# yinan-codes/Rossby-wave-ray-tracing

Measured on AMD Instinct MI355X. Metric: ray-steps/sec (whole node), 10^6 rays RKF45; max |Δpos| vs CPU ref, higher is better.
Workload: dtype f64

## Files before the change

### include/rwrt.h

```cpp
#ifndef RWRT_H
#define RWRT_H

#include <stdint.h>

#ifdef __cplusplus
extern "C" {
#endif

#define RWRT_ABI_VERSION 5
#define RWRT_NFIELD_REF 18
#define RWRT_NFIELD_PACK 12
#define RWRT_NVAR 5
#define RWRT_NMERC 12
#define RWRT_NOUT 8
#define RWRT_NSTATE 12

typedef enum {
  RWRT_OK = 0,
  RWRT_ERR_ARG = 1,
  RWRT_ERR_HIP = 2,
  RWRT_SOLVER_FAILED = 3
} rwrt_status;

typedef struct {
// ... 87 lines not shown
                                int64_t nray, const rwrt_params* p,
                                const double* d_tbound, int32_t it_begin,
                                int32_t it_end, const int64_t* d_order,
                                int64_t n_heavy, double* d_state, int64_t* d_count,
                                int32_t* d_nanrow, double* d_out, int32_t* d_tail_from,
                                double* d_tail_row, int32_t* d_work, void* stream);
rwrt_status rwrt_expand_tails(int64_t nray, int32_t it_begin, int32_t it_end,
                              const int32_t* d_tail_from, const double* d_tail_row,
                              double* d_out, void* stream);

rwrt_status rwrt_row_slots(int64_t nray, const double* d_state, int32_t* d_row_slot, int64_t* d_nslot,
                           void* stream);
rwrt_status rwrt_rk45_run_slots(rwrt_ctx* ctx, const rwrt_grid* g, const double* d_packed,
                                int64_t nray, const rwrt_params* p,
                                const double* d_tbound, int32_t it_begin,
                                int32_t it_end, const int64_t* d_order,
                                int64_t n_heavy, double* d_state, int64_t* d_count,
                                int32_t* d_nanrow, double* d_out, const int32_t* d_row_slot,
                                int32_t* d_tail_from, double* d_tail_row, int32_t* d_work,
                                void* stream);
rwrt_status rwrt_expand_slots(int64_t nray, int32_t it_begin, int32_t it_end, const int32_t* d_row_slot,
                              const int32_t* d_tail_from, const double* d_tail_row, const double* d_rows,
                              double* d_out, void* stream);

typedef struct {
  int32_t nx, ny, nchan, wcol;
  double inv_dlon;
  double lat0, inv_dlat;
} rwrt_density_map;

rwrt_status rwrt_ray_density(const rwrt_density_map* m, int64_t nray,
                             int32_t it_begin, int32_t it_end,
                             const double* d_rows, const int32_t* d_row_slot,
                             const int32_t* d_tail_from, const double* d_tail_row,
                             const int32_t* d_chan, int64_t* d_count, double* d_wsum,
                             void* stream);

#define RWRT_SUMMARY_MAXREG 8
#define RWRT_SUMMARY_NF64 9
#define RWRT_SUMMARY_NI32 4
typedef struct {
  int32_t nreg, reserved;
  double box[RWRT_SUMMARY_MAXREG][4];
} rwrt_summary_regions;

rwrt_status rwrt_ray_summary(int64_t nray, int32_t it_begin, int32_t it_end,
// ... 143 lines not shown
```

### rossby-wave-ray-tracing_amd/_hip.py

```python
import ctypes
import os

import torch

_HERE = os.path.dirname(os.path.abspath(__file__))
LIB_PATH = os.environ.get("RWRT_LIB", os.path.join(_HERE, "librwrt.so"))

NFIELD_REF, NFIELD_PACK, NVAR, NMERC, NOUT, NSTATE = 18, 12, 5, 12, 8, 12
ABI_SYMBOLS = ("rwrt_version", "rwrt_last_error", "rwrt_ctx_create", "rwrt_ctx_destroy",
               "rwrt_ctx_set_latency_density", "rwrt_ctx_set_tv_lanes", "rwrt_ctx_set_handoff",
               "rwrt_ctx_set_trace",
               "rwrt_pack_fields",
               "rwrt_mercator_point", "rwrt_rhs", "rwrt_dp54_attempt",
               "rwrt_ray_initial", "rwrt_rk45_init", "rwrt_rk45_run", "rwrt_rk45_run_tails",
               "rwrt_expand_tails", "rwrt_row_slots", "rwrt_rk45_run_slots", "rwrt_expand_slots",
               "rwrt_rk4_run", "rwrt_ray_density", "rwrt_ray_summary", "rwrt_ray_arrival", "rwrt_ray_flux",
               "rwrt_ray_track", "rwrt_ray_cross",
               "rwrt_wn_map", "rwrt_wn_fill",
               "rwrt_sh_filter",
               "rwrt_bs_ready", "rwrt_bs_diag", "rwrt_rk45_init_tv", "rwrt_rk45_run_tv", "rwrt_rk45_run_tv_tails",
               "rwrt_rk45_run_tv_slots", "rwrt_rhs_tv",
               "rwrt_kat_rk45", "rwrt_selftest_math", "rwrt_host_fill_rows")

RWRT_OK, RWRT_ERR_ARG, RWRT_ERR_HIP, RWRT_SOLVER_FAILED = 0, 1, 2, 3


class RwrtError(RuntimeError):
    pass


class SolverFailed(RwrtError):
    """rkf45.py:423-425: every retrying column has a NaN step (status -1)."""


class Grid(ctypes.Structure):
    _fields_ = [("ncol", ctypes.c_int32), ("nrow", ctypes.c_int32),
                ("lon0", ctypes.c_double), ("dlon", ctypes.c_double),
                ("lat0", ctypes.c_double), ("dlat", ctypes.c_double)]


class Params(ctypes.Structure):
    _fields_ = [("rtol", ctypes.c_double), ("atol", ctypes.c_double),
                ("min_step", ctypes.c_double), ("cut_off", ctypes.c_double),
                ("nt", ctypes.c_int32), ("reserved", ctypes.c_int32),
                ("tstep", ctypes.c_double)]


# ... 76 lines not shown
    lib.rwrt_last_error.restype = ctypes.c_char_p
    G, Pr, B = ctypes.POINTER(Grid), ctypes.POINTER(Params), ctypes.POINTER(Background)
    M = ctypes.POINTER(DensityMap)
    R = ctypes.POINTER(SummaryRegions)
    A = ctypes.POINTER(ArrivalMap)
    F = ctypes.POINTER(FluxMapC)
    T = ctypes.POINTER(TrackMapC)
    X = ctypes.POINTER(CrossMapC)
    sig = {
        "rwrt_pack_fields": [G, _P, _P, _P],
        "rwrt_mercator_point": [G, _P, _I64, _P, _P, _P, _P],
        "rwrt_rhs": [G, _P, _I64, _P, _P, _P],
        "rwrt_dp54_attempt": [G, _P, _I64, _P, _P, _P, _D, _D, _P, _P, _P, _P],
        "rwrt_ray_initial": [G, _P, _I64, _P, _P, _P, _I32, _P, _P, _P, _P],
        "rwrt_rk45_init": [G, _P, _I64, _P, Pr, _P, _P, _P, _P, _P, _P],
        "rwrt_rk45_run": [_P, G, _P, _I64, Pr, _P, _I32, _I32, _P, _I64, _P, _P, _P, _P, _P, _P],
        "rwrt_rk45_run_tails": [_P, G, _P, _I64, Pr, _P, _I32, _I32, _P, _I64, _P, _P, _P, _P, _P, _P, _P,
                                _P],
        "rwrt_expand_tails": [_I64, _I32, _I32, _P, _P, _P, _P],
        "rwrt_row_slots": [_I64, _P, _P, _P, _P],
        "rwrt_rk45_run_slots": [_P, G, _P, _I64, Pr, _P, _I32, _I32, _P, _I64, _P, _P, _P, _P, _P, _P, _P,
                                _P, _P],
        "rwrt_expand_slots": [_I64, _I32, _I32, _P, _P, _P, _P, _P, _P],
        "rwrt_rk4_run": [_P, G, _P, _I64, Pr, _I32, _I32, _P, _P, _P, _P, _P, _P, _P],
        "rwrt_ray_density": [M, _I64, _I32, _I32, _P, _P, _P, _P, _P, _P, _P, _P],
        "rwrt_ray_arrival": [A, _I64, _I32, _I32, _P, _P, _P, _P, _P, _P, _P, _P, _P],
        "rwrt_ray_flux": [F, _I64, _I32, _I32, _P, _P, _P, _P, _P, _P, _P, _P],
        "rwrt_ray_track": [T, _I64, _I32, _I32, _P, _P, _P, _P, _P, _I64, _P, _P, _P, _P, _P, _P, _P],
        "rwrt_ray_cross": [X, _I64, _I32, _I32, _P, _P, _P, _P, _P, _I64, _P, _P, _P, _P, _P, _P, _P, _P, _P],
        "rwrt_ray_summary": [_I64, _I32, _I32, _P, _P, _P, _P, _P, _I64, R, _P, _P, _P],
        "rwrt_wn_map": [G, _P, _I32, _I64, _I32, _P, _P, _P, _I32, _P, _P, _P, _P, _P, _P, _P],
        "rwrt_wn_fill": [_I32, _I32, _I32, _I32, _P, _P, _P],
        "rwrt_sh_filter": [_I32, _I32, _I32, _I32, _P, _P, _P, _P, _P, _P, _P, _P],
        "rwrt_bs_ready": [_I32, _I32, _P, _P, _P, _D, _D, _P, _P, _I32, _P],
        "rwrt_bs_diag": [_I32, _I32, _I32, _P, _P, _P, _D, _D, ctypes.c_uint32, _P, _P, _I32, _P],
        "rwrt_rk45_init_tv": [G, B, _I64, _P, Pr, _P, _P, _P, _P, _P, _P],
        "rwrt_rk45_run_tv": [_P, G, B, _I64, Pr, _P, _I32, _I32, _P, _I64, _P, _P, _P, _P, _P, _P],
        "rwrt_rk45_run_tv_tails": [_P, G, B, _I64, Pr, _P, _I32, _I32, _P, _I64, _P, _P, _P, _P, _P, _P, _P,
                                   _P],
        "rwrt_rk45_run_tv_slots": [_P, G, B, _I64, Pr, _P, _I32, _I32, _P, _I64, _P, _P, _P, _P, _P, _P, _P,
                                   _P, _P],
        "rwrt_ctx_create": [_I32, ctypes.POINTER(_P)],
        "rwrt_ctx_destroy": [_P],
        "rwrt_ctx_set_latency_density": [_P, _I32],
        "rwrt_ctx_set_tv_lanes": [_P, _I32],
        "rwrt_ctx_set_handoff": [_P, _I32],
# ... 61 lines not shown

    def set_latency_density(self, rays_per_wave):
        if getattr(self, "_qpw", 16) != int(rays_per_wave):
            check(load().rwrt_ctx_set_latency_density(self._h, int(rays_per_wave)))
            self._qpw = int(rays_per_wave)

    def set_tv_lanes(self, lanes):
        if getattr(self, "_tvl", 64) != int(lanes):
            check(load().rwrt_ctx_set_tv_lanes(self._h, int(lanes)))
            self._tvl = int(lanes)

    def set_handoff(self, max_rays):
        if getattr(self, "_hof", 16) != int(max_rays):
            check(load().rwrt_ctx_set_handoff(self._h, int(max_rays)))
            self._hof = int(max_rays)

    def set_trace(self, trace=None):
        if trace is None:
            check(load().rwrt_ctx_set_trace(self._h, None, 0))
        else:
            check(load().rwrt_ctx_set_trace(self._h, ctypes.c_void_p(trace.data_ptr()), int(trace.shape[0])))
        self._trace = trace

    def close(self):
        h, self._h = getattr(self, "_h", None), None
        if h is not None and h.value and _lib is not None:
            _lib.rwrt_ctx_destroy(h)

    def __del__(self):
        try:
            self.close()
        except Exception:
            pass
```

### rossby-wave-ray-tracing_amd/csrc/rwrt.hip

```cpp

#include <hip/hip_runtime.h>

#include <cmath>
#include <cstdint>
#include <cstdlib>
#include <cstdio>
#include <cstring>
#include <mutex>
#include <string>
#include <type_traits>

#include "rwrt.h"
#include "nproots.h"

#ifdef RWRT_ANALYZE_HOT
__device__ __forceinline__ bool rwrt_rare_sink(bool c) {
  asm volatile("; rare %0" ::"s"(__builtin_amdgcn_ballot_w64(c)));
  return false;
}
#define RARE(c) rwrt_rare_sink(c)
#else
#define RARE(c) (c)
#endif
#ifdef RWRT_ANALYZE_MARK
// ... 2036 lines not shown
  double cut_a;
  const uint8_t* frozen;
  int32_t quad_per_wave = 16;
  int64_t* trace = nullptr;
  int64_t trace_cap = 0;
  const int32_t* row_slot = nullptr;
  int32_t handoff = 16;
};

template <class BG>
__device__ __forceinline__ double* row_block(const RunArgs<BG>& a, int64_t ray) {
  const int64_t slot = a.row_slot ? (int64_t)a.row_slot[ray] : ray;
  return slot < 0 ? nullptr : a.out + (size_t)slot * (size_t)(a.it_end - a.it_begin) * RWRT_NOUT;
}


__device__ __forceinline__ void store_tail(double* tail_row, int64_t ray, double2 r0, double2 r1, double2 r2,
                                           double2 r3) {
  double2* o = reinterpret_cast<double2*>(tail_row + (size_t)ray * RWRT_NOUT);
  o[0] = r0;
  o[1] = r1;
  o[2] = r2;
  o[3] = r3;
}

constexpr int kTraceWords = 10;
__device__ __forceinline__ void trace_start(int64_t* tr, int64_t w) {
  tr[w * kTraceWords + 3] = (int64_t)__builtin_amdgcn_s_memrealtime();
  tr[w * kTraceWords + 8] = (int64_t)__builtin_amdgcn_s_memtime();
}
__device__ __forceinline__ void trace_ray(int64_t* tr, int64_t w, int64_t ray, int64_t attempts, bool latency) {
  const unsigned hw = __builtin_amdgcn_s_getreg(4 | (31 << 11));
  const unsigned xcc = __builtin_amdgcn_s_getreg(20 | (15 << 11));
  int64_t* r = tr + w * kTraceWords;
  r[0] = ray;
  r[1] = hw;
  r[2] = xcc;
  r[4] = (int64_t)__builtin_amdgcn_s_memrealtime();
  r[5] = attempts;
  r[6] = latency ? 1 : 0;
  r[7] = blockIdx.x;
  r[9] = (int64_t)__builtin_amdgcn_s_memtime();
}

inline double haversine_cut(double cut_off) {
  if (!(cut_off > 0.0 && cut_off <= 3.0)) return -1.0;
// ... 327 lines not shown
      ug = aux[0];
      vg = aux[1];
    } else {
      ugvg_at(a.B, tb, y[0], y[1], y[2], y[3], ug, vg);
    }
    const int last = (st == 2) ? a.it_end : it + 1;
    if (writer && rows) {
      const double2 r0 = make_double2(y[0], y[1]), r1 = make_double2(y[2], y[3]);
      const double2 r2 = make_double2(y[4], ug), r3 = make_double2(vg, (double)nacc);
      for (int kr = it; kr < last; ++kr) {
        double2* o = reinterpret_cast<double2*>(rows + (size_t)(kr - a.it_begin) * RWRT_NOUT);
        store_row16<RWRT_ROW_NT>(o + 0, r0);
        store_row16<RWRT_ROW_NT>(o + 1, r1);
        store_row16<RWRT_ROW_NT>(o + 2, r2);
        store_row16<RWRT_ROW_NT>(o + 3, r3);
      }
    }
    if (nanrow == a.nt && isnan(y[0])) nanrow = it;
    prev_lon = y[0];
    prev_lat = y[1];
    cos_prev = cos_c;
    it = last;
    if (st == 2) t = a.tbound[a.it_end - 1];
    if (it == a.it_end) break;
  }
  if (writer) {
#pragma unroll
    for (int v = 0; v < 5; ++v) {
      a.state[v * a.nray + ray] = y[v];
      a.state[(5 + v) * a.nray + ray] = f[v];
    }
    a.state[10 * a.nray + ray] = t;
    a.state[11 * a.nray + ray] = habs;
    a.count[2 * ray] = nacc;
    a.count[2 * ray + 1] = nrej;
    a.nanrow[ray] = nanrow;
    if (kTrace && w < a.trace_cap) trace_ray(a.trace, w, ray, nacc + nrej - att0, true);
  }
}

template <bool kTrace>
__device__ __forceinline__ void quad_rays(const RunArgs<StaticBG>& a, char* cache, double* Kq, int lb) {
  const CachedStaticBG B = LaneBG<StaticBG>::make(a.B, cache);
  QuadRole R;
  R.role = threadIdx.x & 3;
  R.odd = (R.role & 1) != 0;
  R.high = (R.role & 2) != 0;
// ... 140 lines not shown
      double2* o = reinterpret_cast<double2*>(rows + (size_t)(it - a.it_begin) * RWRT_NOUT);
      store_row16<RWRT_ROW_NT>(o + 0, r0);
      store_row16<RWRT_ROW_NT>(o + 1, r1);
      store_row16<RWRT_ROW_NT>(o + 2, r2);
      store_row16<RWRT_ROW_NT>(o + 3, r3);
    }
    if (RARE(last > it + 1) && writer && rows) {
      asm volatile("");
      for (int k = it + 1; k < last; ++k) {
        double2* o = reinterpret_cast<double2*>(rows + (size_t)(k - a.it_begin) * RWRT_NOUT);
        o[0] = r0;
        o[1] = r1;
        o[2] = r2;
        o[3] = r3;
      }
    }
    if (nanrow == a.nt && isnan(y[0])) nanrow = it;
    prev_lon = y[0];
    prev_lat = y[1];
    cos_prev = cos_c;
    it = last;
    if (st == Lane<RayProblem, KStore>::kFrozen) L.t = a.tbound[a.it_end - 1];
    if (it == a.it_end && writer) {
#pragma unroll
      for (int v = 0; v < 5; ++v) {
        a.state[v * a.nray + ray] = y[v];
        a.state[(5 + v) * a.nray + ray] = L.f[v];
      }
      a.state[10 * a.nray + ray] = L.t;
      a.state[11 * a.nray + ray] = L.habs;
      if (kTrace && wpos < a.trace_cap)
        trace_ray(a.trace, wpos, ray, nacc + nrej - a.count[2 * ray] - a.count[2 * ray + 1], false);
      a.count[2 * ray] = nacc;
      a.count[2 * ray + 1] = nrej;
      a.nanrow[ray] = nanrow;
      ray = -1;
    }
    if ((kReplica || kPair) && it == a.it_end) ray = -1;
    MARK("x_row_end_done");
  }
  if constexpr (kHandoff) {
    const uint64_t hm = __builtin_amdgcn_ballot_w64(handoff);
    if (RARE(hm != 0)) {
      const int q = (int)((threadIdx.x & 63u) >> 2);
      const int nq = __builtin_popcountll(hm);
      uint64_t m = hm;
// ... 64 lines not shown
      run_rays<BG, BBG, false, true>(a, BBG::make(a.B, smem + kKBytes), smem, w);
      return;
    }
  }
  if constexpr (std::is_same<BG, VaryingBG<double>>::value) {
#ifdef RWRT_ANALYZE_PAIR
    if (true) {
#else
    if (a.B.half) {
#endif
      run_rays<BG, PairVaryingBG64, false, false, true>(a, PairVaryingBG64::make(a.B, smem + kKBytes), smem, -1);
      return;
    }
  }
  if constexpr (kLean)
    run_rays<BG, LeanCachedStaticBG, kTrace, false>(a, LeanCachedStaticBG{LaneBG<BG>::make(a.B, smem + kKBytes)}, smem,
                                                    -1);
  else
    run_rays<BG, typename LaneBG<BG>::type, kTrace, false>(a, LaneBG<BG>::make(a.B, smem + kKBytes), smem, -1);
}

__global__ void frozen_flag_kernel(const double* __restrict__ state, int64_t nray,
                                   uint8_t* __restrict__ frozen, int32_t* __restrict__ tail_from = nullptr,
                                   int32_t it_begin = 0, int32_t it_end = 0) {
  for (int64_t i = blockIdx.x * (int64_t)blockDim.x + threadIdx.x; i < nray;
       i += (int64_t)gridDim.x * blockDim.x) {
    double sum = state[i];
#pragma unroll
    for (int v = 1; v < 5; ++v) sum = sum + state[v * nray + i];
    const bool frz = isnan(sum / 5.0);
    frozen[i] = frz ? 1 : 0;
    if (tail_from) tail_from[i] = frz ? it_begin : it_end;
  }
}

constexpr int kFillThreads = 64;
__device__ __forceinline__ void write_frozen_tile(double* out, int64_t base, int64_t nrows, bool mine,
                                                  double2 r0, double2 r1, double2 r2, double2 r3) {
  unsigned long long lanes = __ballot(mine);
  const int64_t nq = nrows * 4;
  const int qt = threadIdx.x & 3;
  while (lanes) {
    const int j = __builtin_ctzll(lanes);
    lanes &= lanes - 1;
    double2* o = reinterpret_cast<double2*>(out + (size_t)(base + j) * nrows * RWRT_NOUT);
    const double2 q0 = make_double2(__shfl(r0.x, j), __shfl(r0.y, j));
    const double2 q1 = make_double2(__shfl(r1.x, j), __shfl(r1.y, j));
// ... 472 lines not shown

struct DeviceGuard {
  int prev = -1;
  bool ok = true;
  explicit DeviceGuard(int dev) {
    if (hipGetDevice(&prev) != hipSuccess) prev = -1;
    if (prev != dev) ok = hipSetDevice(dev) == hipSuccess;
  }
  ~DeviceGuard() {
    int cur = -1;
    if (prev >= 0 && hipGetDevice(&cur) == hipSuccess && cur != prev) (void)hipSetDevice(prev);
  }
};

rwrt_status ctx_flags(rwrt_ctx* c, int64_t nray) {
  if ((size_t)nray <= c->cap) return RWRT_OK;
  if (c->flags) {
    if ((c->used && hipEventSynchronize(c->done) != hipSuccess) || hipFree(c->flags) != hipSuccess)
      return check_launch("releasing the context's frozen-ray flags");
    c->flags = nullptr;
    c->cap = 0;
  }
  const size_t cap = ((size_t)nray + 4095) & ~(size_t)4095;
  if (hipMalloc(reinterpret_cast<void**>(&c->flags), cap) != hipSuccess)
    return fail(RWRT_ERR_HIP, "frozen-ray flag allocation failed%s");
  c->cap = cap;
  return RWRT_OK;
}

rwrt_status ctx_image(rwrt_ctx* c, const Field& F, hipStream_t stream, const char** out,
                      const int** range = nullptr) {
  const size_t image = cache_image_bytes((int64_t)F.W * F.H), need = image + kRangeInts * sizeof(int);
  if (need > c->img_cap) {
    if (c->img) {
      if ((c->used && hipEventSynchronize(c->done) != hipSuccess) || hipFree(c->img) != hipSuccess)
        return check_launch("releasing the context's cache image");
      c->img = nullptr;
      c->img_cap = 0;
    }
    if (hipMalloc(reinterpret_cast<void**>(&c->img), need) != hipSuccess)
      return fail(RWRT_ERR_HIP, "cache image allocation failed%s");
    c->img_cap = need;
  }
  int* r = reinterpret_cast<int*>(c->img + image);
  if (hipMemsetAsync(r, 0, kRangeInts * sizeof(int), stream) != hipSuccess)
    return check_launch("hipMemsetAsync(exponent range)");
  hipLaunchKernelGGL(cache_image_kernel, dim3(grid_for((int64_t)F.W * F.H * 6, 256)), dim3(256), 0, stream,
// ... 68 lines not shown
  const int32_t quad_per_wave = ctx->quad_per_wave;
  const int32_t handoff = ctx->handoff;
  const int64_t per_block = BG::kTimeVarying ? 4 : 4 * (int64_t)quad_per_wave;
  const int64_t team_blocks = (n_heavy + per_block - 1) / per_block;
  if (team_blocks > ctx->ncu / 2)
    return fail(RWRT_ERR_ARG, "n_heavy exceeds the latency mode's capacity (per CU 4 x rays-per-wave, time-varying 4; half the CUs)%s");
  DeviceGuard dg(ctx->device);
  if (!dg.ok) return check_launch("hipSetDevice(context device)");
  hipStream_t st = (hipStream_t)stream;
  if (hipMemsetAsync(d_work, 0, 2 * sizeof(int32_t), st) != hipSuccess)
    return check_launch("hipMemsetAsync(queue)");
  int64_t blocks = ctx_persistent_blocks<BG>(ctx);
  if (team_blocks) blocks = std::max<int64_t>(1, blocks - team_blocks * (blocks / ctx->ncu));
  int64_t block_rays = 256;
  if constexpr (BG::kTimeVarying) block_rays = B.half ? 128 : 256;
  const int64_t need = (nray - n_heavy + block_rays - 1) / block_rays;
  if (blocks > need) blocks = need;
  RunArgs<BG> a{B, nray, p->rtol, p->atol, p->min_step, p->cut_off, p->nt, it_begin, it_end,
                d_tbound, d_order, d_state, d_count, d_nanrow, d_out, d_work,
                n_heavy, 0, haversine_cut(p->cut_off), nullptr};
  a.row_slot = d_row_slot;
  a.handoff = handoff;
  if (rwrt_status s = ctx_flags(ctx, nray)) return s;
  a.frozen = ctx->flags;
  if (rwrt_status s = ctx_begin(ctx, st, [&] {
        hipLaunchKernelGGL(frozen_flag_kernel, dim3(grid_for(nray, 256)), dim3(256), 0, st, d_state, nray,
                           ctx->flags, d_tail_from, it_begin, it_end);
      }))
    return s;
  if constexpr (std::is_same<BG, StaticBG>::value) {
    if (rwrt_status s = ctx_image(ctx, B.F, st, &a.B.img, &a.B.range)) return s;
  }
  a.heavy_blocks = (int32_t)team_blocks;
  a.quad_per_wave = quad_per_wave;
  if constexpr (std::is_same<BG, StaticBG>::value) {
    a.trace = ctx->trace;
    a.trace_cap = ctx->trace ? ctx->trace_cap : 0;
  }
  if (nray > n_heavy || team_blocks) {
    const int64_t grid = team_blocks + (nray > n_heavy ? blocks : 0);
    if (a.trace && std::is_same<BG, StaticBG>::value) {
      if constexpr (std::is_same<BG, StaticBG>::value) {
        hipLaunchKernelGGL((rk45_run_kernel<BG, true>), dim3((unsigned)grid), dim3(256), 0, st, a);
        hipLaunchKernelGGL((rk45_run_kernel<BG, true, true>), dim3((unsigned)grid), dim3(256), 0, st, a);
      }
    } else {
      hipLaunchKernelGGL(rk45_run_kernel<BG>, dim3((unsigned)grid), dim3(256), 0, st, a);
      if constexpr (std::is_same<BG, StaticBG>::value)
        hipLaunchKernelGGL((rk45_run_kernel<BG, false, true>), dim3((unsigned)grid), dim3(256), 0, st, a);
    }
// ... 748 lines not shown
```

### rossby-wave-ray-tracing_amd/engine.py

```python
import os

import numpy as np
import torch

import _hip as H
from constants import rearth as R_EARTH
from launch_rows import deliver

F64 = torch.float64


def grid_of(lon, lat, ncol):
    lon = np.asarray(lon, np.float64)
    lat = np.asarray(lat, np.float64)
    return H.Grid(int(ncol), len(lat), float(lon[0]), float(lon[1] - lon[0]),
                  float(lat[0]), float(lat[1] - lat[0]))


def t_eval_of(nt, tstep, ttotal=None):
    t = np.arange(nt) * np.float64(tstep)
    if ttotal is not None and t[-1] > ttotal:
        t[-1] = ttotal
    return t


class RunResult:

    def __init__(self, nacc, nrej, nanrow, failed, break_row, n_live):
        self.nacc = nacc
        self.nrej = nrej
        self.nanrow = nanrow
        self.failed = failed
        self.break_row = break_row
        self.n_live = n_live
        self.bounds = []

    @property
    def ray_steps(self):
        return int(self.nacc.sum().item())


class Tails:

    def __init__(self, nray, device):
        self.frm = torch.empty(nray, dtype=torch.int32, device=device)
        self.row = torch.empty((nray, H.NOUT), dtype=F64, device=device)

    def take(self, idx):
        t = Tails.__new__(Tails)
        t.frm, t.row = self.frm[idx].contiguous(), self.row[idx].contiguous()
        return t

    def last_row(self, view, i1):
        return torch.where((self.frm < i1)[:, None], self.row, view[:, -1])


class Slots:

    def __init__(self, nray, device):
        self.slot = torch.empty(nray, dtype=torch.int32, device=device)
        self.n_dev = torch.zeros(1, dtype=torch.int64, device=device)
        self.n = None

    def compute(self, st, stream):
        H.check(H.load().rwrt_row_slots(st["nray"], H.dptr(st["state"]), H.dptr(self.slot, torch.int32),
                                        H.dptr(self.n_dev, torch.int64), stream))
        return self

    def count(self):
        self.n = int(self.n_dev.item())
        return self.n

    def last_row(self, view, tails, i1):
        blk = view[self.slot.clamp(min=0).to(torch.int64), -1] if view.shape[0] else tails.row
        return torch.where((tails.frm < i1)[:, None], tails.row, blk)

    def dense(self, view, tails, i0, i1, out=None):
        nray = self.slot.numel()
        if out is None or out.numel() < nray * (i1 - i0) * H.NOUT:
            out = torch.empty((nray, i1 - i0, H.NOUT), dtype=F64, device=self.slot.device)
        d = out.reshape(-1)[: nray * (i1 - i0) * H.NOUT].view(nray, i1 - i0, H.NOUT)
        H.check(H.load().rwrt_expand_slots(nray, int(i0), int(i1), H.dptr(self.slot, torch.int32),
                                           H.dptr(tails.frm, torch.int32), H.dptr(tails.row, F64),
                                           H.dptr(view, F64), H.dptr(d, F64), H.stream(self.slot.device)))
        return d


class RayEngine:

    use_tails = os.environ.get("RWRT_TAILS", "1") != "0"
    tv_lanes = int(os.environ.get("RWRT_TV_LANES", "32"))
    use_slots = os.environ.get("RWRT_SLOTS", "1") != "0"
    handoff = int(os.environ.get("RWRT_HANDOFF", "16"))

    def __init__(self, fields, lon, lat, device=None):
        H.require_gpu()
        H.load()
        self.device = torch.device(device or "cuda")
        f = torch.as_tensor(np.ascontiguousarray(fields, dtype=np.float64)) \
            if not torch.is_tensor(fields) else fields.to(F64)
        if f.ndim != 3 or f.shape[-1] != H.NFIELD_REF:
            raise ValueError(f"fields must be [ncol, nrow, {H.NFIELD_REF}], got {tuple(f.shape)}")
        f = f.to(self.device).contiguous()
        self.grid = grid_of(lon, lat, f.shape[0])
        self.lon, self.lat = np.array(lon, np.float64), np.array(lat, np.float64)
        self.packed = torch.empty((f.shape[0], f.shape[1], H.NFIELD_PACK), dtype=F64,
                                  device=self.device)
        H.check(H.load().rwrt_pack_fields(self.grid, H.dptr(f), H.dptr(self.packed), self._stream()))
        self.work = torch.zeros(4, dtype=torch.int32, device=self.device)

    bg = None
    split_rho = None
    launch_log = ()
    rows_bytes = 0
    launch_handoffs = ()

# ... 263 lines not shown
        cum = torch.cumsum(w, 0)
        best = None
        tv = self.bg is not None
        lanes_cu = (4.0 * self.tv_lanes) if (tv and self.bg.fp32 == 0) else 256.0
        for q in ((1,) if tv else self.QUAD_DENSITIES):
            cap = min((ncu // 2) * 4 * q, n_live)
            n = torch.arange(0, cap + 1, 4 * q, device=w.device)
            n = torch.unique(torch.cat([n, torch.tensor([cap], device=w.device)]))
            rest = cum[-1] - torch.where(n > 0, cum[(n - 1).clamp(min=0)], torch.zeros_like(cum[:1]))
            lanes = lanes_cu * (ncu - (n + 4 * q - 1) // (4 * q)).clamp(min=1)
            nxt = torch.where(n < w.numel(), w[n.clamp(max=w.numel() - 1)], torch.zeros_like(rest))
            ratio = self.TV_RATIO if tv else \
                self.QUAD_RATIO_1 + (self.QUAD_RATIO_16 - self.QUAD_RATIO_1) * (q - 1) / 15.0
            t = torch.maximum(torch.maximum(nxt, rest / lanes),
                              torch.where(n > 0, w[0] * ratio, torch.zeros_like(rest)))
            k = int(torch.argmin(t).item())
            cand = (float(t[k]), int(n[k].item()), q, float(t[0]))
            if best is None or cand[0] < best[0] - 1e-9 * best[0]:
                best = cand
        t_best, n_best, q_best, t_none = best
        if n_best == 0 or t_best > (1.0 - self.QUAD_MIN_GAIN) * t_none:
            return 0, 16
        return n_best, q_best

    def run(self, st, p, tbound, it_begin, it_end, out, order=None, n_heavy=0, rays_per_wave=16, tails=None,
            slots=None):
        lib = H.load()
        ctx = self.ctx
        if self.bg is not None:
            ctx.set_tv_lanes(self.tv_lanes)
        if n_heavy:
            ctx.set_latency_density(rays_per_wave)
        ctx.set_handoff(self.handoff)
        if slots is not None and tails is None:
            raise ValueError("row slots need tails")
        if self.bg is None:
            fn, bg = (lib.rwrt_rk45_run if tails is None else lib.rwrt_rk45_run_tails if slots is None
                      else lib.rwrt_rk45_run_slots), H.dptr(self.packed)
        else:
            fn, bg = (lib.rwrt_rk45_run_tv if tails is None else lib.rwrt_rk45_run_tv_tails if slots is None
                      else lib.rwrt_rk45_run_tv_slots), ctypes_ref(self.bg)
        args = [ctx.handle, self.grid, bg, st["nray"], ctypes_ref(p), H.dptr(tbound, F64),
                int(it_begin), int(it_end), H.dptr(order, torch.int64), int(n_heavy),
                H.dptr(st["state"]), H.dptr(st["count"]), H.dptr(st["nanrow"]), H.dptr(out, F64)]
        if slots is not None:
            args += [H.dptr(slots.slot, torch.int32)]
# ... 131 lines not shown
            i0 = bounds[-1][1]
        rows_max = max([b - a for a, b in bounds] or [1])
        use_slots = (self.use_slots and self.use_tails and nray > 0
                     and (getattr(sink, "takes_slots", False) or (sink is None and out is None)))
        sbufs = None
        nblk = nray
        if use_slots:
            first = Slots(nray, self.device).compute(st, self._stream())
            nblk = max(1, first.count())
        bufs = _row_buffers(out, nblk, rows_max, self.device)
        self.rows_bytes = sum(b.numel() for b in bufs) * 8
        tbufs = [self.tails(nray) for _ in bufs]
        if use_slots:
            sbufs = [first] + [Slots(nray, self.device) for _ in bufs[1:]]
        order = None
        if prev_work is None or order_policy not in ("cost", "priority", "cell", "total"):
            order = self.live_first_order_of(st)
        works = []
        self.split_rho = None
        auto_split, split_rows = self.parse_split(split)
        self.launch_log = []
        self.launch_handoffs = []
        self.launch_work = []
        k = 0
        while k < len(bounds):
            i0, i1 = bounds[k]
            if (auto_split and k == n_lead and len(works) == 2 and i1 - i0 > 2 * split_rows[0]
                    and order_policy in ("cost", "priority", "total")):
                live = ~torch.isnan(st["state"][:5].sum(0))
                rho = self.rank_corr(works[0], works[1], live)
                self.split_rho = rho
                if rho < self.SPLIT_RHO:
                    bounds[k:k + 1] = self.cut_bounds(i0, i1, split_rows)
                    i1 = bounds[k][1]
                    order_policy = "total"
                if os.environ.get("RWRT_DEBUG_SCHED"):
                    print(f"split: rank correlation {rho:.3f} -> {'split' if rho < self.SPLIT_RHO else 'one launch'}",
                          flush=True)
            flat = bufs[k % len(bufs)].view(-1)
            view = flat[: nblk * (i1 - i0) * H.NOUT].view(nblk, i1 - i0, H.NOUT)
            slots = None
            if sbufs is not None:
                slots = sbufs[k % len(sbufs)]
                if k > 0:
                    slots.compute(st, self._stream())
            work = None
            if order_policy in ("cost", "priority", "cell", "total") and prev_work is not None:
                work = cnt.sum(1) - (0 if order_policy == "total" else prev_work)
            tk = team[min(k, len(team) - 1)] if isinstance(team, list) else team
            if order_policy in ("cost", "priority", "cell", "total") and prev_work is not None:
                head = (self.team_capacity_tv() if self.bg is not None else self.team_capacity()) if tk else 0
                order = (self.cost_cell_order(st, work, head=head)
                         if order_policy == "cell" else self.cost_order(st, work))
            n_heavy, qpw = self.team_size(tk, st, work, order, i1 - i0) if tk else (0, 16)
            self.launch_log.append({"rows": [int(i0), int(i1)], "n_heavy": int(n_heavy), "per_wave": int(qpw)})
            if os.environ.get("RWRT_DEBUG_TEAM"):
                print(f"launch rows [{i0}, {i1}): n_heavy {n_heavy} at {qpw} per wave", flush=True)
            prev_work = cnt.sum(1)
            tails = tbufs[k % len(bufs)]
            if events is not None:
                e0, e1, es = self._event_pair()
                self.run(st, p, tb, i0, i1, view, order, n_heavy, qpw, tails, slots)
                e1.record(es)
                events.append((e0, e1))
            else:
                self.run(st, p, tb, i0, i1, view, order, n_heavy, qpw, tails, slots)
            self.launch_handoffs.append(self.work[0:1].clone())
            if auto_split and k < n_lead:
                works = (works + [cnt.sum(1) - prev_work])[-2:]
            if self.keep_launch_work:
                self.launch_work.append((cnt.sum(1) - prev_work, order[:n_heavy].clone() if n_heavy else None))
            if sink is not None:
                deliver(self, sink, i0, i1, view, tails, slots)
            elif tails is not None and out is not None:
                self.expand(view, tails, i0, i1)
            k += 1
        mx = int(st["nanrow"].max().item()) if nray else 0
        if group is not None:
            from shard import reduce_max
            mx = reduce_max(mx, group)
        brk = mx if mx < nt else None
# ... 128 lines not shown
```

### rossby-wave-ray-tracing_amd/shard.py

```python
import time

import numpy as np
import torch
import torch.distributed as dist


COLLECTIVE_MIN_WORLD = 2


def collective(world):
    return world >= COLLECTIVE_MIN_WORLD


def world_info(group=None):
    if not (dist.is_available() and dist.is_initialized()):
        return 0, 1
    return dist.get_rank(group), dist.get_world_size(group)


def _dev(group=None):
    if dist.is_initialized() and dist.get_backend(group) == "nccl":
        return torch.device("cuda", torch.cuda.current_device())
    return torch.device("cpu")

# ... 212 lines not shown
        else:
            cost, frozen = costs
            sh = probe_share(nray, rank, world, eng.device)
            sub = eng.take(st, sh)
            eng.run(sub, p, tb, 1, 1 + npr, torch.empty((sh.numel(), npr, 8), dtype=torch.float64,
                                                         device=eng.device),
                    eng.live_first_order_of(sub), 0, tails=eng.tails(sh.numel()))
        idx = cost_partition(cost, frozen, rank, world)
        local = eng.take(st, idx)
        prow = torch.empty((idx.numel(), npr, 8), dtype=torch.float64, device=eng.device)
        ptails = eng.tails(idx.numel())
        eng.run(local, p, tb, 1, 1 + npr, prow, eng.live_first_order_of(local), 0, tails=ptails)
        prow_local, ptails_local = prow, ptails
        if events is not None:
            e1.record(es)
            events.append((e0, e1))
    else:
        prow = torch.empty((nray, npr, 8), dtype=torch.float64, device=eng.device)
        ptails = eng.tails(nray)
        eng.run(st, p, tb, 1, 1 + npr, prow, eng.live_first_order_of(st), 0, tails=ptails)
        if events is not None:
            e1.record(es)
            events.append((e0, e1))
        cost = st["count"].sum(1)
        frozen = torch.isnan(st["state"][:5].sum(0))
        idx = cost_partition(cost, frozen, rank, world)
        local = eng.take(st, idx)
        prow_local, ptails_local = prow[idx], None if ptails is None else ptails.take(idx)
    last = {}

    dense = {}

    def keep(i0, i1, rows, tails=None, slots=None):
        if slots is not None:
            last["row"] = slots.last_row(rows, tails, i1)
        else:
            last["row"] = rows[:, -1] if tails is None else tails.last_row(rows, i1)
        if sink is not None:
            deliver(eng, sink, i0, i1, rows, tails, slots, idx=idx, scratch=dense)
    keep.takes_tails = True
    keep.takes_slots = True

    keep(1, 1 + npr, prow_local, ptails_local)
    n_live_local = int((~frozen[idx]).sum().item())
    res = eng.advance(local, p, tb, 1 + npr, chunk=chunk, sink=keep, out=out, events=events,
                      group=group, order_policy=order_policy, first_chunk=list(lead),
                      n_live=int(summary[0]), n_live_local=n_live_local,
                      prev_work=torch.zeros_like(cost[idx]), team=team, split=split)
    steps_local = int(local["count"][:, 0].sum().item())
    ends = cnts = None
    if gather:
        end_row = last["row"].clone()
        if group is not None and collective(world):
            ends = gather_rows(end_row, idx.cpu().numpy(), nray, group=group)
            cnts = gather_rows(local["count"], idx.cpu().numpy(), nray, group=group)
        else:
            ends, cnts = end_row, local["count"]
    return ShardedRun(idx, res, steps_local, ends, cnts)
```

Before: 4.038 billion.

## Fuse per-launch cost ordering into a native plan kernel with radix sort

```diff
diff --git a/include/rwrt.h b/include/rwrt.h
--- a/include/rwrt.h
+++ b/include/rwrt.h
@@ -133,6 +133,14 @@
 rwrt_status rwrt_expand_slots(int64_t nray, int32_t it_begin, int32_t it_end, const int32_t* d_row_slot,
                               const int32_t* d_tail_from, const double* d_tail_row, const double* d_rows,
                               double* d_out, void* stream);
+
+#define RWRT_PLAN_SINCE 0
+#define RWRT_PLAN_TOTAL 1
+rwrt_status rwrt_launch_plan_bytes(int64_t nray, int64_t* bytes);
+rwrt_status rwrt_launch_plan(int64_t nray, int32_t policy, const double* d_state,
+                             const int64_t* d_count, int64_t* d_prev_work, int64_t* d_work,
+                             int64_t* d_order, int32_t* d_row_slot, int64_t* d_nslot,
+                             int64_t* h_nlive, void* d_scratch, int64_t scratch_bytes, void* stream);
 
 typedef struct {
   int32_t nx, ny, nchan, wcol;
diff --git a/rossby-wave-ray-tracing_amd/_hip.py b/rossby-wave-ray-tracing_amd/_hip.py
--- a/rossby-wave-ray-tracing_amd/_hip.py
+++ b/rossby-wave-ray-tracing_amd/_hip.py
@@ -14,6 +14,7 @@
                "rwrt_mercator_point", "rwrt_rhs", "rwrt_dp54_attempt",
                "rwrt_ray_initial", "rwrt_rk45_init", "rwrt_rk45_run", "rwrt_rk45_run_tails",
                "rwrt_expand_tails", "rwrt_row_slots", "rwrt_rk45_run_slots", "rwrt_expand_slots",
+               "rwrt_launch_plan_bytes", "rwrt_launch_plan",
                "rwrt_rk4_run", "rwrt_ray_density", "rwrt_ray_summary", "rwrt_ray_arrival", "rwrt_ray_flux",
                "rwrt_ray_track", "rwrt_ray_cross",
                "rwrt_wn_map", "rwrt_wn_fill",
@@ -23,6 +24,7 @@
                "rwrt_kat_rk45", "rwrt_selftest_math", "rwrt_host_fill_rows")
 
 RWRT_OK, RWRT_ERR_ARG, RWRT_ERR_HIP, RWRT_SOLVER_FAILED = 0, 1, 2, 3
+PLAN_SINCE, PLAN_TOTAL = 0, 1
 
 
 class RwrtError(RuntimeError):
@@ -145,6 +147,8 @@
         "rwrt_rk45_run_slots": [_P, G, _P, _I64, Pr, _P, _I32, _I32, _P, _I64, _P, _P, _P, _P, _P, _P, _P,
                                 _P, _P],
         "rwrt_expand_slots": [_I64, _I32, _I32, _P, _P, _P, _P, _P, _P],
+        "rwrt_launch_plan_bytes": [_I64, ctypes.POINTER(_I64)],
+        "rwrt_launch_plan": [_I64, _I32, _P, _P, _P, _P, _P, _P, _P, ctypes.POINTER(_I64), _P, _I64, _P],
         "rwrt_rk4_run": [_P, G, _P, _I64, Pr, _I32, _I32, _P, _P, _P, _P, _P, _P, _P],
         "rwrt_ray_density": [M, _I64, _I32, _I32, _P, _P, _P, _P, _P, _P, _P, _P],
         "rwrt_ray_arrival": [A, _I64, _I32, _I32, _P, _P, _P, _P, _P, _P, _P, _P, _P],
@@ -252,6 +256,24 @@
             check(load().rwrt_ctx_set_trace(self._h, ctypes.c_void_p(trace.data_ptr()), int(trace.shape[0])))
         self._trace = trace
 
+    _plan_scratch = None
+    _plan_rays = 0
+
+    def launch_plan(self, nray, total, state, count, prev_work, work, order, row_slot, nslot):
+        lib = load()
+        if self._plan_scratch is None or self._plan_rays < nray:
+            need = _I64()
+            check(lib.rwrt_launch_plan_bytes(int(nray), ctypes.byref(need)))
+            self._plan_scratch = torch.empty(need.value, dtype=torch.uint8, device=self.device)
+            self._plan_rays = int(nray)
+        n_live = _I64()
+        i64 = torch.int64
+        check(lib.rwrt_launch_plan(int(nray), PLAN_TOTAL if total else PLAN_SINCE, dptr(state), dptr(count, i64),
+                                   dptr(prev_work, i64), dptr(work, i64), dptr(order, i64),
+                                   dptr(row_slot, torch.int32), dptr(nslot, i64), ctypes.byref(n_live),
+                                   dptr(self._plan_scratch), self._plan_scratch.numel(), stream(self.device)))
+        return int(n_live.value)
+
     def close(self):
         h, self._h = getattr(self, "_h", None), None
         if h is not None and h.value and _lib is not None:
diff --git a/rossby-wave-ray-tracing_amd/csrc/plan.hip b/rossby-wave-ray-tracing_amd/csrc/plan.hip
--- /dev/null
+++ b/rossby-wave-ray-tracing_amd/csrc/plan.hip
@@ -0,0 +1,241 @@
+#include <hip/hip_runtime.h>
+
+#include <cstdint>
+#include <cstring>
+
+#include <rocprim/device/device_radix_sort.hpp>
+
+#include "abi_host.h"
+
+namespace rwrt {
+namespace {
+
+constexpr int kPlanTile = 4096;
+constexpr size_t kPlanAlign = 256;
+constexpr size_t kPlanMergeLimit = 64 * 1024;
+using PlanSort = rocprim::radix_sort_config<rocprim::default_config, rocprim::default_config,
+                                            rocprim::default_config, kPlanMergeLimit>;
+
+struct PlanHead {
+  unsigned long long max_key;
+  long long n_live;
+};
+
+struct PlanLayout {
+  size_t tile, head, keys_in, vals_in, keys_out, temp, temp_bytes, total;
+};
+
+size_t plan_up(size_t x) { return (x + kPlanAlign - 1) & ~(kPlanAlign - 1); }
+
+hipError_t plan_sort_bytes(size_t n, size_t* bytes) {
+  return rocprim::radix_sort_pairs_desc<PlanSort>(
+      nullptr, *bytes, static_cast<unsigned long long*>(nullptr), static_cast<unsigned long long*>(nullptr),
+      static_cast<int64_t*>(nullptr), static_cast<int64_t*>(nullptr), n, 0u, 64u, (hipStream_t) nullptr);
+}
+
+hipError_t plan_layout(int64_t nray, PlanLayout* L) {
+  const size_t n = (size_t)nray, tiles = (n + kPlanTile - 1) / kPlanTile;
+  size_t temp = 0, merge = 0;
+  hipError_t e = plan_sort_bytes(n, &temp);
+  if (e == hipSuccess) e = plan_sort_bytes(n < kPlanMergeLimit ? n : kPlanMergeLimit, &merge);
+  if (e != hipSuccess) return e;
+  temp = merge > temp ? merge : temp;
+  L->tile = 0;
+  L->head = plan_up(tiles * sizeof(int32_t));
+  L->keys_in = L->head + plan_up(sizeof(PlanHead));
+  L->vals_in = L->keys_in + plan_up(n * 8);
+  L->keys_out = L->vals_in + plan_up(n * 8);
+  L->temp = L->keys_out + plan_up(n * 8);
+  L->temp_bytes = plan_up(temp);
+  L->total = L->temp + L->temp_bytes;
+  return hipSuccess;
+}
+
+__device__ __forceinline__ bool plan_live(const double* __restrict__ state, int64_t nray, int64_t i) {
+  double sum = state[i];
+#pragma unroll
+  for (int v = 1; v < 5; ++v) sum = sum + state[v * nray + i];
+  return !isnan(sum / 5.0);
+}
+
+__global__ void __launch_bounds__(256)
+plan_count_kernel(const double* __restrict__ state, const int64_t* __restrict__ count,
+                  int64_t* __restrict__ prev_work, int64_t* __restrict__ work, int64_t nray, int total,
+                  int32_t* __restrict__ tile_count, PlanHead* __restrict__ head) {
+  const int64_t base = (int64_t)blockIdx.x * kPlanTile;
+  int c = 0;
+  unsigned long long mx = 0;
+  for (int k = 0; k < kPlanTile / 256; ++k) {
+    const int64_t i = base + k * 256 + threadIdx.x;
+    if (i < nray) {
+      const int64_t all = count[2 * i] + count[2 * i + 1];
+      const int64_t w = total ? all : all - prev_work[i];
+      work[i] = w;
+      prev_work[i] = all;
+      if (plan_live(state, nray, i)) {
+        ++c;
+        const unsigned long long key = (unsigned long long)w;
+        mx = key > mx ? key : mx;
+      }
+    }
+  }
+  __shared__ int part[4];
+  __shared__ unsigned long long pmax[4];
+  for (int o = 32; o > 0; o >>= 1) {
+    c += __shfl_xor(c, o);
+    const unsigned long long other = __shfl_xor(mx, o);
+    mx = other > mx ? other : mx;
+  }
+  if ((threadIdx.x & 63) == 0) {
+    part[threadIdx.x >> 6] = c;
+    pmax[threadIdx.x >> 6] = mx;
+  }
+  __syncthreads();
+  if (threadIdx.x == 0) {
+    tile_count[blockIdx.x] = part[0] + part[1] + part[2] + part[3];
+    for (int w = 1; w < 4; ++w) mx = pmax[w] > mx ? pmax[w] : mx;
+    if (mx) atomicMax(&head->max_key, mx);
+  }
+}
+
+__global__ void __launch_bounds__(1024)
+plan_offsets_kernel(int64_t tiles, int32_t* __restrict__ tile_count, PlanHead* __restrict__ head,
+                    int64_t* __restrict__ nslot) {
+  __shared__ int wsum[16];
+  __shared__ int carry;
+  if (threadIdx.x == 0) carry = 0;
+  __syncthreads();
+  const int lane = threadIdx.x & 63, wave = threadIdx.x >> 6;
+  for (int64_t t0 = 0; t0 < tiles; t0 += 1024) {
+    const int64_t t = t0 + threadIdx.x;
+    const int v = t < tiles ? tile_count[t] : 0;
+    int x = v;
+    for (int o = 1; o < 64; o <<= 1) {
+      const int y = __shfl_up(x, o);
+      if (lane >= o) x += y;
+    }
+    if (lane == 63) wsum[wave] = x;
+    __syncthreads();
+    int before = carry;
+    for (int w = 0; w < wave; ++w) before += wsum[w];
+    if (t < tiles) tile_count[t] = before + x - v;
+    __syncthreads();
+    if (threadIdx.x == 1023) carry = before + x;
+    __syncthreads();
+  }
+  if (threadIdx.x == 0) {
+    head->n_live = carry;
+    *nslot = carry;
+  }
+}
+
+__global__ void __launch_bounds__(256)
+plan_assign_kernel(const double* __restrict__ state, const int64_t* __restrict__ work, int64_t nray,
+                   const int32_t* __restrict__ tile_off, const PlanHead* __restrict__ head,
+                   int32_t* __restrict__ row_slot, unsigned long long* __restrict__ keys,
+                   int64_t* __restrict__ vals, int64_t* __restrict__ order) {
+  const int64_t base = (int64_t)blockIdx.x * kPlanTile;
+  __shared__ int off;
+  __shared__ int wcnt[4];
+  if (threadIdx.x == 0) off = tile_off[blockIdx.x];
+  __syncthreads();
+  const int64_t n_live = head->n_live;
+  const int lane = threadIdx.x & 63, wave = threadIdx.x >> 6;
+  for (int k = 0; k < kPlanTile / 256; ++k) {
+    const int64_t i = base + k * 256 + threadIdx.x;
+    const bool live = i < nray && plan_live(state, nray, i);
+    const uint64_t m = __ballot(live);
+    if (lane == 0) wcnt[wave] = __popcll(m);
+    __syncthreads();
+    int before = off;
+    for (int w = 0; w < wave; ++w) before += wcnt[w];
+    const int mine = before + __popcll(m & ((1ull << lane) - 1ull));
+    if (i < nray) {
+      row_slot[i] = live ? mine : -1;
+      if (live) {
+        keys[mine] = (unsigned long long)work[i];
+        vals[mine] = i;
+      } else {
+        order[n_live + (i - mine)] = i;
+      }
+    }
+    __syncthreads();
+    if (threadIdx.x == 0) off += wcnt[0] + wcnt[1] + wcnt[2] + wcnt[3];
+    __syncthreads();
+  }
+}
+
+bool misaligned(const void* p, size_t a) { return reinterpret_cast<uintptr_t>(p) % a != 0; }
+
+}
+}
+
+using namespace rwrt;
+
+extern "C" rwrt_status rwrt_launch_plan_bytes(int64_t nray, int64_t* bytes) {
+  if (!bytes) return fail(RWRT_ERR_ARG, "rwrt_launch_plan_bytes: bytes is NULL%s", "");
+  if (nray < 0 || nray > 0x7fffffffLL) return fail(RWRT_ERR_ARG, "rwrt_launch_plan_bytes: nray out of range%s", "");
+  PlanLayout L;
+  if (const hipError_t e = plan_layout(nray, &L))
+    return fail(RWRT_ERR_HIP, "rwrt_launch_plan_bytes: sort storage query: %s", hipGetErrorString(e));
+  *bytes = (int64_t)L.total;
+  return RWRT_OK;
+}
+
+extern "C" rwrt_status rwrt_launch_plan(int64_t nray, int32_t policy, const double* d_state,
+                                        const int64_t* d_count, int64_t* d_prev_work, int64_t* d_work,
+                                        int64_t* d_order, int32_t* d_row_slot, int64_t* d_nslot,
+                                        int64_t* h_nlive, void* d_scratch, int64_t scratch_bytes, void* stream) {
+  if (nray < 0 || nray > 0x7fffffffLL) return fail(RWRT_ERR_ARG, "rwrt_launch_plan: nray out of range%s", "");
+  if (policy != RWRT_PLAN_SINCE && policy != RWRT_PLAN_TOTAL)
+    return fail(RWRT_ERR_ARG, "rwrt_launch_plan: unknown policy (RWRT_PLAN_SINCE or RWRT_PLAN_TOTAL)%s", "");
+  if (!d_nslot || !h_nlive) return fail(RWRT_ERR_ARG, "rwrt_launch_plan: NULL d_nslot or h_nlive%s", "");
+  if (nray > 0 && (!d_state || !d_count || !d_prev_work || !d_work || !d_order || !d_row_slot || !d_scratch))
+    return fail(RWRT_ERR_ARG, "rwrt_launch_plan: NULL buffer%s", "");
+  if (misaligned(d_state, 8) || misaligned(d_count, 8) || misaligned(d_prev_work, 8) || misaligned(d_work, 8) ||
+      misaligned(d_order, 8) || misaligned(d_nslot, 8) || misaligned(d_row_slot, 4) ||
+      misaligned(d_scratch, kPlanAlign))
+    return fail(RWRT_ERR_ARG, "rwrt_launch_plan: misaligned buffer (d_scratch: 256 bytes)%s", "");
+  hipStream_t st = (hipStream_t)stream;
+  if (nray == 0) {
+    *h_nlive = 0;
+    if (hipMemsetAsync(d_nslot, 0, sizeof(int64_t), st) != hipSuccess) return check_launch("hipMemsetAsync(nslot)");
+    return RWRT_OK;
+  }
+  PlanLayout L;
+  if (const hipError_t e = plan_layout(nray, &L))
+    return fail(RWRT_ERR_HIP, "rwrt_launch_plan: sort storage query: %s", hipGetErrorString(e));
+  if (scratch_bytes < (int64_t)L.total)
+    return fail(RWRT_ERR_ARG, "rwrt_launch_plan: d_scratch is smaller than rwrt_launch_plan_bytes asks%s", "");
+  char* s = static_cast<char*>(d_scratch);
+  int32_t* tile = reinterpret_cast<int32_t*>(s + L.tile);
+  PlanHead* head = reinterpret_cast<PlanHead*>(s + L.head);
+  unsigned long long* keys_in = reinterpret_cast<unsigned long long*>(s + L.keys_in);
+  int64_t* vals_in = reinterpret_cast<int64_t*>(s + L.vals_in);
+  unsigned long long* keys_out = reinterpret_cast<unsigned long long*>(s + L.keys_out);
+  const int64_t tiles = (nray + kPlanTile - 1) / kPlanTile;
+  if (hipMemsetAsync(head, 0, sizeof(PlanHead), st) != hipSuccess) return check_launch("hipMemsetAsync(plan head)");
+  hipLaunchKernelGGL(plan_count_kernel, dim3((unsigned)tiles), dim3(256), 0, st, d_state, d_count, d_prev_work,
+                     d_work, nray, policy == RWRT_PLAN_TOTAL ? 1 : 0, tile, head);
+  hipLaunchKernelGGL(plan_offsets_kernel, dim3(1), dim3(1024), 0, st, tiles, tile, head, d_nslot);
+  hipLaunchKernelGGL(plan_assign_kernel, dim3((unsigned)tiles), dim3(256), 0, st, d_state, d_work, nray, tile, head,
+                     d_row_slot, keys_in, vals_in, d_order);
+  if (rwrt_status e = check_launch("plan kernels")) return e;
+  PlanHead h;
+  if (hipMemcpyAsync(&h, head, sizeof(PlanHead), hipMemcpyDeviceToHost, st) != hipSuccess ||
+      hipStreamSynchronize(st) != hipSuccess)
+    return check_launch("rwrt_launch_plan: reading the live count back");
+  *h_nlive = h.n_live;
+  if (h.n_live > 0) {
+    unsigned bits = 1;
+    while (bits < 64 && (h.max_key >> bits) != 0) ++bits;
+    size_t temp = 0;
+    if (plan_sort_bytes((size_t)h.n_live, &temp) != hipSuccess || temp > L.temp_bytes)
+      return fail(RWRT_ERR_HIP, "rwrt_launch_plan: the sort's storage exceeds the scratch's share%s", "");
+    temp = L.temp_bytes;
+    const hipError_t e = rocprim::radix_sort_pairs_desc<PlanSort>(s + L.temp, temp, keys_in, keys_out, vals_in, d_order,
+                                                                 (size_t)h.n_live, 0u, bits, st);
+    if (e != hipSuccess) return fail(RWRT_ERR_HIP, "rwrt_launch_plan: radix sort: %s", hipGetErrorString(e));
+  }
+  return check_launch("rwrt_launch_plan");
+}
diff --git a/rossby-wave-ray-tracing_amd/csrc/rwrt.hip b/rossby-wave-ray-tracing_amd/csrc/rwrt.hip
--- a/rossby-wave-ray-tracing_amd/csrc/rwrt.hip
+++ b/rossby-wave-ray-tracing_amd/csrc/rwrt.hip
@@ -2082,6 +2082,12 @@
   o[1] = r1;
   o[2] = r2;
   o[3] = r3;
+}
+
+constexpr int kFlagHead = 256;
+template <class BG>
+__device__ __forceinline__ double* last_rows(const RunArgs<BG>& a) {
+  return *reinterpret_cast<double* const*>(a.frozen - kFlagHead);
 }
 
 constexpr int kTraceWords = 10;
@@ -2455,7 +2461,14 @@
     cos_prev = cos_c;
     it = last;
     if (st == 2) t = a.tbound[a.it_end - 1];
-    if (it == a.it_end) break;
+    if (it == a.it_end) {
+      if (writer) {
+        if (double* const lr = last_rows(a))
+          store_tail(lr, ray, make_double2(y[0], y[1]), make_double2(y[2], y[3]), make_double2(y[4], ug),
+                     make_double2(vg, (double)nacc));
+      }
+      break;
+    }
   }
   if (writer) {
 #pragma unroll
@@ -2642,6 +2655,7 @@
     it = last;
     if (st == Lane<RayProblem, KStore>::kFrozen) L.t = a.tbound[a.it_end - 1];
     if (it == a.it_end && writer) {
+      if (double* const lr = last_rows(a)) store_tail(lr, ray, r0, r1, r2, r3);
 #pragma unroll
       for (int v = 0; v < 5; ++v) {
         a.state[v * a.nray + ray] = y[v];
@@ -2752,7 +2766,8 @@
 
 __global__ void frozen_flag_kernel(const double* __restrict__ state, int64_t nray,
                                    uint8_t* __restrict__ frozen, int32_t* __restrict__ tail_from = nullptr,
-                                   int32_t it_begin = 0, int32_t it_end = 0) {
+                                   int32_t it_begin = 0, int32_t it_end = 0, double* tail_row = nullptr) {
+  if (blockIdx.x == 0 && threadIdx.x == 0) *reinterpret_cast<double**>(frozen - kFlagHead) = tail_row;
   for (int64_t i = blockIdx.x * (int64_t)blockDim.x + threadIdx.x; i < nray;
        i += (int64_t)gridDim.x * blockDim.x) {
     double sum = state[i];
@@ -3271,7 +3286,7 @@
     c->cap = 0;
   }
   const size_t cap = ((size_t)nray + 4095) & ~(size_t)4095;
-  if (hipMalloc(reinterpret_cast<void**>(&c->flags), cap) != hipSuccess)
+  if (hipMalloc(reinterpret_cast<void**>(&c->flags), cap + kFlagHead) != hipSuccess)
     return fail(RWRT_ERR_HIP, "frozen-ray flag allocation failed%s");
   c->cap = cap;
   return RWRT_OK;
@@ -3386,10 +3401,10 @@
   a.row_slot = d_row_slot;
   a.handoff = handoff;
   if (rwrt_status s = ctx_flags(ctx, nray)) return s;
-  a.frozen = ctx->flags;
+  a.frozen = ctx->flags + kFlagHead;
   if (rwrt_status s = ctx_begin(ctx, st, [&] {
         hipLaunchKernelGGL(frozen_flag_kernel, dim3(grid_for(nray, 256)), dim3(256), 0, st, d_state, nray,
-                           ctx->flags, d_tail_from, it_begin, it_end);
+                           ctx->flags + kFlagHead, d_tail_from, it_begin, it_end, d_tail_row);
       }))
     return s;
   if constexpr (std::is_same<BG, StaticBG>::value) {
diff --git a/rossby-wave-ray-tracing_amd/engine.py b/rossby-wave-ray-tracing_amd/engine.py
--- a/rossby-wave-ray-tracing_amd/engine.py
+++ b/rossby-wave-ray-tracing_amd/engine.py
@@ -40,6 +40,9 @@
         return int(self.nacc.sum().item())
 
 
+LAST_ROWS = os.environ.get("RWRT_LAST_ROWS", "1") != "0"
+
+
 class Tails:
 
     def __init__(self, nray, device):
@@ -52,6 +55,8 @@
         return t
 
     def last_row(self, view, i1):
+        if LAST_ROWS:
+            return self.row
         return torch.where((self.frm < i1)[:, None], self.row, view[:, -1])
 
 
@@ -72,6 +77,8 @@
         return self.n
 
     def last_row(self, view, tails, i1):
+        if LAST_ROWS:
+            return tails.row
         blk = view[self.slot.clamp(min=0).to(torch.int64), -1] if view.shape[0] else tails.row
         return torch.where((tails.frm < i1)[:, None], tails.row, blk)
 
@@ -92,6 +99,7 @@
     tv_lanes = int(os.environ.get("RWRT_TV_LANES", "32"))
     use_slots = os.environ.get("RWRT_SLOTS", "1") != "0"
     handoff = int(os.environ.get("RWRT_HANDOFF", "16"))
+    use_plan = os.environ.get("RWRT_PLAN", "1") != "0"
 
     def __init__(self, fields, lon, lat, device=None):
         H.require_gpu()
@@ -401,6 +409,18 @@
         if n_best == 0 or t_best > (1.0 - self.QUAD_MIN_GAIN) * t_none:
             return 0, 16
         return n_best, q_best
+
+    def team_fixed(self, team, n_live):
+        if self.bg is not None and self.bg.fp32 == 2:
+            return 0, 16
+        ncu = torch.cuda.get_device_properties(self.device).multi_processor_count
+        n, q = (int(team[0]), int(team[1])) if isinstance(team, (tuple, list)) else (int(team), 16)
+        return min(n, (ncu // 2) * 4 * (1 if self.bg is not None else q), n_live), q
+
+    def plan_buffers(self, nray):
+        return {"work": torch.empty(nray, dtype=torch.int64, device=self.device),
+                "order": torch.empty(nray, dtype=torch.int64, device=self.device),
+                "slots": Slots(nray, self.device)}
 
     def run(self, st, p, tbound, it_begin, it_end, out, order=None, n_heavy=0, rays_per_wave=16, tails=None,
             slots=None):
@@ -578,6 +598,7 @@
         self.launch_log = []
         self.launch_handoffs = []
         self.launch_work = []
+        plan, own_prev = None, False
         k = 0
         while k < len(bounds):
             i0, i1 = bounds[k]
@@ -595,24 +616,32 @@
                           flush=True)
             flat = bufs[k % len(bufs)].view(-1)
             view = flat[: nblk * (i1 - i0) * H.NOUT].view(nblk, i1 - i0, H.NOUT)
-            slots = None
-            if sbufs is not None:
-                slots = sbufs[k % len(sbufs)]
-                if k > 0:
+            slots = sbufs[k % len(sbufs)] if sbufs is not None else None
+            tk = team[min(k, len(team) - 1)] if isinstance(team, list) else team
+            costed = order_policy in ("cost", "priority", "cell", "total") and prev_work is not None
+            work = None
+            if costed and self.use_plan and order_policy != "cell" and tk != "auto" and nray > 0:
+                plan = plan or self.plan_buffers(nray)
+                if not own_prev:
+                    prev_work, own_prev = prev_work.clone(), True
+                work, order = plan["work"], plan["order"]
+                ps = slots if slots is not None else plan["slots"]
+                ps.n = self.ctx.launch_plan(nray, order_policy == "total", st["state"], cnt, prev_work, work,
+                                            order, ps.slot, ps.n_dev)
+                n_heavy, qpw = self.team_fixed(tk, ps.n) if tk else (0, 16)
+            else:
+                if slots is not None and k > 0:
                     slots.compute(st, self._stream())
-            work = None
-            if order_policy in ("cost", "priority", "cell", "total") and prev_work is not None:
-                work = cnt.sum(1) - (0 if order_policy == "total" else prev_work)
-            tk = team[min(k, len(team) - 1)] if isinstance(team, list) else team
-            if order_policy in ("cost", "priority", "cell", "total") and prev_work is not None:
-                head = (self.team_capacity_tv() if self.bg is not None else self.team_capacity()) if tk else 0
-                order = (self.cost_cell_order(st, work, head=head)
-                         if order_policy == "cell" else self.cost_order(st, work))
-            n_heavy, qpw = self.team_size(tk, st, work, order, i1 - i0) if tk else (0, 16)
+                if costed:
+                    work = cnt.sum(1) - (0 if order_policy == "total" else prev_work)
+                    head = (self.team_capacity_tv() if self.bg is not None else self.team_capacity()) if tk else 0
+                    order = (self.cost_cell_order(st, work, head=head)
+                             if order_policy == "cell" else self.cost_order(st, work))
+                n_heavy, qpw = self.team_size(tk, st, work, order, i1 - i0) if tk else (0, 16)
+                prev_work, own_prev = cnt.sum(1), True
             self.launch_log.append({"rows": [int(i0), int(i1)], "n_heavy": int(n_heavy), "per_wave": int(qpw)})
             if os.environ.get("RWRT_DEBUG_TEAM"):
                 print(f"launch rows [{i0}, {i1}): n_heavy {n_heavy} at {qpw} per wave", flush=True)
-            prev_work = cnt.sum(1)
             tails = tbufs[k % len(bufs)]
             if events is not None:
                 e0, e1, es = self._event_pair()
diff --git a/rossby-wave-ray-tracing_amd/shard.py b/rossby-wave-ray-tracing_amd/shard.py
--- a/rossby-wave-ray-tracing_amd/shard.py
+++ b/rossby-wave-ray-tracing_amd/shard.py
@@ -258,11 +258,15 @@
         if events is not None:
             e1.record(es)
             events.append((e0, e1))
-        cost = st["count"].sum(1)
         frozen = torch.isnan(st["state"][:5].sum(0))
-        idx = cost_partition(cost, frozen, rank, world)
-        local = eng.take(st, idx)
-        prow_local, ptails_local = prow[idx], None if ptails is None else ptails.take(idx)
+        if world == 1:
+            idx = torch.arange(nray, device=eng.device)
+            local, prow_local, ptails_local = st, prow, ptails
+        else:
+            cost = st["count"].sum(1)
+            idx = cost_partition(cost, frozen, rank, world)
+            local = eng.take(st, idx)
+            prow_local, ptails_local = prow[idx], None if ptails is None else ptails.take(idx)
     last = {}
 
     dense = {}
@@ -278,11 +282,12 @@
     keep.takes_slots = True
 
     keep(1, 1 + npr, prow_local, ptails_local)
-    n_live_local = int((~frozen[idx]).sum().item())
+    n_live_local = int((~(frozen if world == 1 else frozen[idx])).sum().item())
     res = eng.advance(local, p, tb, 1 + npr, chunk=chunk, sink=keep, out=out, events=events,
                       group=group, order_policy=order_policy, first_chunk=list(lead),
                       n_live=int(summary[0]), n_live_local=n_live_local,
-                      prev_work=torch.zeros_like(cost[idx]), team=team, split=split)
+                      prev_work=torch.zeros(idx.numel(), dtype=torch.int64, device=eng.device), team=team,
+                      split=split)
     steps_local = int(local["count"][:, 0].sum().item())
     ends = cnts = None
     if gather:
```

Result: faster. 4.218 billion (median of 6 runs) (+4.5%).
